# arangesh/TrackMPNN

Hardware: AMD Instinct MI355X
Metric: graph_edges_per_sec_fwd_bwd (higher is better)
Workload: dtype f32; 1 GPU; C2 KITTI Car/RRC-shaped rolling windows: 7 frames, D_t~clip(Poisson(6),1,20), F=8 (2d), H=64, K=0, diff; 1 fwd per frame + 1 bwd per window; 16384 windows/GPU batched block-diagonally (64 distinct seeds tiled); windows_per_gpu=16384, rows_final=6762496, parallelism=sequence-dp1

## Files before the change

### trackmpnn_amd/csrc/intf.hip

```cpp
#include "common.h"
#include <stdlib.h>

namespace tmpnn {

static constexpr float IT_EPS = 1e-5f;
static constexpr int IT_CH = 128;
static constexpr int IT_SPB = 32;
static constexpr int IT_FMAX = 128;
static constexpr int IT_NT = 1024;

struct ItFwdArgs {
    const float* x; const int64_t* x_rows; int ld_x; int F; int nd;
    const int32_t* seg_ptr; const int32_t* seg_cnt; const int32_t* seg_of_det; int S; int training;
    const float* w1; const float* b1; const float* gamma; const float* beta;
    const float* run_mean; const float* run_var; const float* w2; const float* b2;
    float* y_save; float* mean; float* rstd; const int32_t* out_row; float* h_new; int ld_h;
};

__device__ __forceinline__ int it_chunk_end(const int* s_sp, int s0, int sa, int s1) {
    const int base = s_sp[sa - s0];
    int sb = sa + 1;
    while (sb < s1 && s_sp[sb + 1 - s0] - base <= IT_CH) ++sb;
    return sb;
}

template <int H>
__global__ __launch_bounds__(IT_NT) void k_it_fwd(ItFwdArgs a) {
    constexpr int NSUB = IT_NT / H, LD = H + 4;
    extern __shared__ __attribute__((aligned(16))) float it_lds[];
    float* s_w2 = it_lds;
    float* s_y = s_w2 + H * LD;
    float* s_a = s_y + IT_CH * LD;
    float* s_mean = s_a + IT_CH * LD;
    float* s_rstd = s_mean + IT_SPB * H;
    float* s_w1 = s_rstd + IT_SPB * H;
    float* s_x = s_w1;
    const int tid = threadIdx.x, c = tid % H, sub = tid / H;
    const int F = a.F;
    for (int i = tid; i < H * H; i += IT_NT) s_w2[(i / H) * LD + (i % H)] = a.w2[i];
    float w1r[16];
    if (F <= 16) {
#pragma unroll
        for (int f = 0; f < 16; ++f) w1r[f] = f < F ? a.w1[c * F + f] : 0.f;
    } else {
        for (int i = tid; i < H * F; i += IT_NT) s_w1[(i / F) * (F + 1) + (i % F)] = a.w1[i];
    }
    const float b1 = a.b1[c], gam = a.gamma[c], bet = a.beta[c], b2 = a.b2[c];
    __shared__ int s_sp[IT_SPB + 1];
    if (!a.training) {
        if (sub == 0) {
            const float m = a.run_mean[c], r = rsqrtf(a.run_var[c] + IT_EPS);
            s_mean[c] = m; s_rstd[c] = r;
            if (blockIdx.x == 0) { a.mean[c] = m; a.rstd[c] = r; }
        }
    }
    const int ngroups = a.training ? (a.S + IT_SPB - 1) / IT_SPB : (a.nd + IT_CH - 1) / IT_CH;
    for (int grp = blockIdx.x; grp < ngroups; grp += gridDim.x) {
    int s0, s1;
    if (a.training) { s0 = grp * IT_SPB; s1 = min(a.S, s0 + IT_SPB); }
    else { s0 = grp; s1 = s0 + 1; }
    __syncthreads();
    if (a.training && tid <= s1 - s0) s_sp[tid] = a.seg_ptr[s0 + tid];
    __syncthreads();
    for (int sa = s0; sa < s1;) {
        int sb, ra, rb;
        if (a.training) { sb = it_chunk_end(s_sp, s0, sa, s1); ra = s_sp[sa - s0]; rb = s_sp[sb - s0]; }
        else { sb = s1; ra = sa * IT_CH; rb = min(a.nd, ra + IT_CH); }
        const int nr = rb - ra;
        if (F <= 16) {
            for (int t = tid; t < nr * 16; t += IT_NT) {
                const int i = t >> 4, f = t & 15;
                const size_t xrow = a.x_rows ? (size_t)a.x_rows[ra + i] : (size_t)(ra + i);
                s_x[t] = f < F ? a.x[xrow * a.ld_x + f] : 0.f;
            }
            __syncthreads();
        }
        for (int i = sub; i < nr; i += NSUB) {
            const float* xr = a.x + ((F > 16 && a.x_rows) ? (size_t)a.x_rows[ra + i] : (size_t)(ra + i)) * a.ld_x;
            float acc = b1;
            if (F <= 16) {
#pragma unroll
                for (int f4 = 0; f4 < 4; ++f4) {
                    const float4 xv = *reinterpret_cast<const float4*>(s_x + i * 16 + 4 * f4);
                    acc = fmaf(xv.x, w1r[4 * f4], acc); acc = fmaf(xv.y, w1r[4 * f4 + 1], acc);
                    acc = fmaf(xv.z, w1r[4 * f4 + 2], acc); acc = fmaf(xv.w, w1r[4 * f4 + 3], acc);
                }
            } else {
                for (int f = 0; f < F; ++f) acc = fmaf(xr[f], s_w1[c * (F + 1) + f], acc);
            }
            s_y[i * LD + c] = acc;
            a.y_save[(size_t)(ra + i) * H + c] = acc;
        }
        __syncthreads();
        if (a.training) {
            for (int s = sa + sub; s < sb; s += NSUB) {
                const int p0 = s_sp[s - s0] - ra, p1 = s_sp[s + 1 - s0] - ra;
                const float cnt = (float)a.seg_cnt[s], nz = cnt - (float)(p1 - p0);
                float sum = nz * b1;
                for (int i = p0; i < p1; ++i) sum += s_y[i * LD + c];
                const float m = sum / cnt;
                float sq = nz * (b1 - m) * (b1 - m);
                for (int i = p0; i < p1; ++i) { const float d = s_y[i * LD + c] - m; sq += d * d; }
                const float r = rsqrtf(sq / cnt + IT_EPS);
                s_mean[(s - sa) * H + c] = m; s_rstd[(s - sa) * H + c] = r;
                a.mean[(size_t)s * H + c] = m; a.rstd[(size_t)s * H + c] = r;
            }
            __syncthreads();
        }
        for (int i = sub; i < nr; i += NSUB) {
            int sl = 0;
            if (a.training) { while (s_sp[sa - s0 + sl + 1] - ra <= i) ++sl; }
            const float yh = (s_y[i * LD + c] - s_mean[sl * H + c]) * s_rstd[sl * H + c];
            s_a[i * LD + c] = fmaxf(yh * gam + bet, 0.f);
        }
        __syncthreads();
        for (int i0 = sub; i0 < nr; i0 += 4 * NSUB) {
            float acc[4] = {b2, b2, b2, b2};
            int rr[4], orow[4];
#pragma unroll
            for (int t = 0; t < 4; ++t) rr[t] = min(i0 + t * NSUB, nr - 1);
#pragma unroll
            for (int t = 0; t < 4; ++t) orow[t] = a.out_row[ra + rr[t]];
#pragma unroll 4
            for (int k4 = 0; k4 < H / 4; ++k4) {
                const float4 w = *reinterpret_cast<const float4*>(s_w2 + c * LD + 4 * k4);
#pragma unroll
                for (int t = 0; t < 4; ++t) {
                    const float4 av = *reinterpret_cast<const float4*>(s_a + rr[t] * LD + 4 * k4);
                    acc[t] = fmaf(av.x, w.x, acc[t]); acc[t] = fmaf(av.y, w.y, acc[t]);
                    acc[t] = fmaf(av.z, w.z, acc[t]); acc[t] = fmaf(av.w, w.w, acc[t]);
                }
            }
#pragma unroll
            for (int t = 0; t < 4; ++t) {
                const int i = i0 + t * NSUB;
                if (i < nr) a.h_new[(size_t)orow[t] * a.ld_h + c] = acc[t];
            }
        }
        __syncthreads();
        sa = sb;
    }
    }
}

struct ItBwdArgs {
    const float* x; const int64_t* x_rows; int ld_x; int F; int nd;
    const int32_t* seg_ptr; const int32_t* seg_cnt; const int32_t* seg_of_det; int S; int training;
    const float* w1; const float* b1; const float* gamma; const float* beta; const float* w2;
    const float* y_save; const float* mean; const float* rstd; const int32_t* out_row;
    const float* d_h; int ld_dh; float* d_xdet; int ld_dx; float* d_xzero;
    float* slabs; int slab_floats;
};

template <int H, int FPT>
__global__ __launch_bounds__(IT_NT) void k_it_bwd(ItBwdArgs a) {
    constexpr int NSUB = IT_NT / H, LD = H + 4, KPT = H / NSUB;
    extern __shared__ __attribute__((aligned(16))) float it_lds[];
    float* s_w2 = it_lds;
    float* s_d = s_w2 + H * LD;
    float* s_a = s_d + IT_CH * LD;
    float* s_yh = s_a + IT_CH * LD;
    float* s_dy0 = s_yh + IT_CH * LD;
    float* s_red = s_dy0 + IT_SPB * H;
    float* s_x = s_red + 4 * IT_NT;
    float* s_w1 = s_x + IT_CH * 16;
    const int tid = threadIdx.x, c = tid % H, sub = tid / H;
    const int F = a.F;
    for (int i = tid; i < H * H; i += IT_NT) s_w2[(i % H) * LD + (i / H)] = a.w2[i];
    if (F <= 16)
        for (int i = tid; i < H * 16; i += IT_NT) s_w1[(i >> 4) * 17 + (i & 15)] = (i & 15) < F ? a.w1[(i >> 4) * F + (i & 15)] : 0.f;
    const float b1 = a.b1[c], gam = a.gamma[c], bet = a.beta[c];
    float acc_w2[KPT];
#pragma unroll
    for (int j = 0; j < KPT; ++j) acc_w2[j] = 0.f;
    float acc_w1[FPT];
#pragma unroll
    for (int j = 0; j < FPT; ++j) acc_w1[j] = 0.f;
    float v_db2 = 0.f, v_dg = 0.f, v_dbt = 0.f, v_db1 = 0.f;
    __shared__ int s_sp[IT_SPB + 1];
    const int ngroups = a.training ? (a.S + IT_SPB - 1) / IT_SPB : (a.nd + IT_CH - 1) / IT_CH;
    for (int grp = blockIdx.x; grp < ngroups; grp += gridDim.x) {
    int s0, s1;
    if (a.training) { s0 = grp * IT_SPB; s1 = min(a.S, s0 + IT_SPB); }
    else { s0 = grp; s1 = s0 + 1; }
    __syncthreads();
    if (a.training && tid <= s1 - s0) s_sp[tid] = a.seg_ptr[s0 + tid];
    __syncthreads();
    for (int sa = s0; sa < s1;) {
        int sb, ra, rb;
        if (a.training) { sb = it_chunk_end(s_sp, s0, sa, s1); ra = s_sp[sa - s0]; rb = s_sp[sb - s0]; }
        else { sb = s1; ra = sa * IT_CH; rb = min(a.nd, ra + IT_CH); }
        const int nr = rb - ra;
        {
            constexpr int RPT = IT_CH / NSUB;
            int orow[RPT], sg[RPT];
#pragma unroll
            for (int j = 0; j < RPT; ++j) {
                const int i = min(sub + j * NSUB, nr - 1);
                orow[j] = a.out_row[ra + i];
                int sl = 0;
                if (a.training) { while (s_sp[sa - s0 + sl + 1] - ra <= i) ++sl; }
                sg[j] = a.training ? sa + sl : 0;
            }
            float dv[RPT], yv[RPT], mv[RPT], rv[RPT];
#pragma unroll
            for (int j = 0; j < RPT; ++j) {
                const int i = min(sub + j * NSUB, nr - 1);
                dv[j] = a.d_h[(size_t)orow[j] * a.ld_dh + c];
                yv[j] = a.y_save[(size_t)(ra + i) * H + c];
                mv[j] = a.mean[(size_t)sg[j] * H + c];
                rv[j] = a.rstd[(size_t)sg[j] * H + c];
            }
#pragma unroll
            for (int j = 0; j < RPT; ++j) {
                const int i = sub + j * NSUB;
                if (i < nr) {
                    const float yh = (yv[j] - mv[j]) * rv[j];
                    s_yh[i * LD + c] = yh;
                    s_a[i * LD + c] = fmaxf(yh * gam + bet, 0.f);
                    s_d[i * LD + c] = dv[j];
                }
            }
        }
        if (F <= 16) {
            for (int t = tid; t < nr * 16; t += IT_NT) {
                const int i = t >> 4, f = t & 15;
                const size_t xrow = a.x_rows ? (size_t)a.x_rows[ra + i] : (size_t)(ra + i);
                s_x[t] = f < F ? a.x[xrow * a.ld_x + f] : 0.f;
            }
        }
        __syncthreads();
#pragma unroll 8
        for (int i = 0; i < nr; ++i) {
            const float d = s_d[i * LD + c];
            if (sub == 0) v_db2 += d;
            if constexpr (KPT % 4 == 0) {
#pragma unroll
                for (int j4 = 0; j4 < KPT / 4; ++j4) {
                    const float4 av = *reinterpret_cast<const float4*>(s_a + i * LD + KPT * sub + 4 * j4);
                    acc_w2[4 * j4 + 0] = fmaf(d, av.x, acc_w2[4 * j4 + 0]); acc_w2[4 * j4 + 1] = fmaf(d, av.y, acc_w2[4 * j4 + 1]);
                    acc_w2[4 * j4 + 2] = fmaf(d, av.z, acc_w2[4 * j4 + 2]); acc_w2[4 * j4 + 3] = fmaf(d, av.w, acc_w2[4 * j4 + 3]);
                }
            } else {
#pragma unroll
                for (int j = 0; j < KPT; ++j) acc_w2[j] = fmaf(d, s_a[i * LD + KPT * sub + j], acc_w2[j]);
            }
        }
        __syncthreads();
        for (int i0 = sub; i0 < nr; i0 += 4 * NSUB) {
            float da[4] = {0.f, 0.f, 0.f, 0.f};
            int rr[4];
#pragma unroll
            for (int t = 0; t < 4; ++t) rr[t] = min(i0 + t * NSUB, nr - 1);
#pragma unroll 4
            for (int c4 = 0; c4 < H / 4; ++c4) {
                const float4 w = *reinterpret_cast<const float4*>(s_w2 + c * LD + 4 * c4);
#pragma unroll
                for (int t = 0; t < 4; ++t) {
                    const float4 dv = *reinterpret_cast<const float4*>(s_d + rr[t] * LD + 4 * c4);
                    da[t] = fmaf(dv.x, w.x, da[t]); da[t] = fmaf(dv.y, w.y, da[t]);
                    da[t] = fmaf(dv.z, w.z, da[t]); da[t] = fmaf(dv.w, w.w, da[t]);
                }
            }
            float dyh[4];
#pragma unroll
            for (int t = 0; t < 4; ++t) {
                const int i = i0 + t * NSUB;
                dyh[t] = 0.f;
                if (i < nr) {
                    const float dz = s_a[i * LD + c] > 0.f ? da[t] : 0.f;
                    v_dg = fmaf(dz, s_yh[i * LD + c], v_dg);
                    v_dbt += dz;
                    dyh[t] = dz * gam;
                }
            }
#pragma unroll
            for (int t = 0; t < 4; ++t) {
                const int i = i0 + t * NSUB;
                if (i < nr) s_a[i * LD + c] = dyh[t];
            }
        }
        __syncthreads();
        if (a.training) {
            for (int s = sa + sub; s < sb; s += NSUB) {
                const int p0 = s_sp[s - s0] - ra, p1 = s_sp[s + 1 - s0] - ra;
                const float cnt = (float)a.seg_cnt[s], nz = cnt - (float)(p1 - p0);
                const float m = a.mean[(size_t)s * H + c], r = a.rstd[(size_t)s * H + c];
                float q1 = 0.f, q2 = 0.f;
                for (int i = p0; i < p1; ++i) { const float g = s_a[i * LD + c]; q1 += g; q2 = fmaf(g, s_yh[i * LD + c], q2); }
                const float inv = 1.0f / cnt;
                for (int i = p0; i < p1; ++i) {
                    const float dy = r * (s_a[i * LD + c] - q1 * inv - s_yh[i * LD + c] * q2 * inv);
                    s_a[i * LD + c] = dy;
                    v_db1 += dy;
                }
                const float yh0 = (b1 - m) * r;
                const float dy0 = r * (-q1 * inv - yh0 * q2 * inv);
                v_db1 = fmaf(nz, dy0, v_db1);
                s_dy0[(s - sa) * H + c] = dy0;
            }
        } else {
            const float r = a.rstd[c];
            for (int i = sub; i < nr; i += NSUB) { const float dy = r * s_a[i * LD + c]; s_a[i * LD + c] = dy; v_db1 += dy; }
        }
        __syncthreads();
        if (F <= 16) {
#pragma unroll 4
            for (int i = 0; i < nr; ++i) {
                const float dy = s_a[i * LD + c];
#pragma unroll
                for (int j = 0; j < (FPT < 4 ? FPT : 4); ++j) {
                    const int f = sub + j * NSUB;
                    if (f < 16) acc_w1[j] = fmaf(dy, s_x[i * 16 + f], acc_w1[j]);
                }
            }
        } else {
            for (int i = 0; i < nr; ++i) {
                const float dy = s_a[i * LD + c];
                const float* xr = a.x + (a.x_rows ? (size_t)a.x_rows[ra + i] : (size_t)(ra + i)) * a.ld_x;
#pragma unroll
                for (int j = 0; j < FPT; ++j) {
                    const int f = sub + j * NSUB;
                    if (f < F) acc_w1[j] = fmaf(dy, xr[f], acc_w1[j]);
                }
            }
        }
        if (a.d_xdet) {
            for (int t = tid; t < nr * F; t += IT_NT) {
                const int i = t / F, f = t - i * F;
                float acc = 0.f;
                if (F <= 16) {
#pragma unroll 8
                    for (int k = 0; k < H; ++k) acc = fmaf(s_a[i * LD + k], s_w1[k * 17 + f], acc);
                } else {
                    for (int k = 0; k < H; ++k) acc = fmaf(s_a[i * LD + k], a.w1[k * F + f], acc);
                }
                a.d_xdet[(size_t)(ra + i) * a.ld_dx + f] = acc;
            }
        }
        if (a.d_xzero && a.training) {
            const int ns = sb - sa;
            for (int t = tid; t < ns * F; t += IT_NT) {
                const int s = t / F, f = t - s * F;
                float acc = 0.f;
                if (F <= 16) {
#pragma unroll 8
                    for (int k = 0; k < H; ++k) acc = fmaf(s_dy0[s * H + k], s_w1[k * 17 + f], acc);
                } else {
                    for (int k = 0; k < H; ++k) acc = fmaf(s_dy0[s * H + k], a.w1[k * F + f], acc);
                }
                a.d_xzero[(size_t)(sa + s) * F + f] = acc;
            }
        }
        __syncthreads();
        sa = sb;
    }
    }
    float* slab = a.slabs + (size_t)blockIdx.x * a.slab_floats;
#pragma unroll
    for (int j = 0; j < KPT; ++j) slab[c * H + KPT * sub + j] = acc_w2[j];
    float* sl_w1 = slab + H * H;
#pragma unroll
    for (int j = 0; j < FPT; ++j) {
        const int f = sub + j * NSUB;
        if (f < F) sl_w1[c * F + f] = acc_w1[j];
    }
    s_red[0 * IT_NT + tid] = v_db2; s_red[1 * IT_NT + tid] = v_dg; s_red[2 * IT_NT + tid] = v_dbt; s_red[3 * IT_NT + tid] = v_db1;
    __syncthreads();
    if (sub == 0) {
        float* sl_v = sl_w1 + H * F;
#pragma unroll
        for (int q = 0; q < 4; ++q) {
            float v = 0.f;
            for (int t = 0; t < NSUB; ++t) v += s_red[q * IT_NT + t * H + c];
            sl_v[q * H + c] = v;
        }
    }
}

static constexpr int ITW_R = 32;
static constexpr int ITW_MS = 8;
static constexpr int ITW_NW = 8;
static constexpr int ITW_SPB = 64;
static constexpr int ITW_FWD_WAVE_FLOATS = ITW_R * 64 + ITW_R * 16;
static constexpr int ITW_BWD_WAVE_FLOATS = 2 * ITW_R * 64 + ITW_R * 16;

#define ITW_LDS_SYNC() asm volatile("s_waitcnt lgkmcnt(0)" ::: "memory")
__device__ __forceinline__ int itw_chunk_end(const int* s_sp, int s0, int sa, int s1) {
    const int base = s_sp[sa - s0];
    int sb = sa + 1;
    while (sb < s1 && sb - sa < ITW_MS && s_sp[sb + 1 - s0] - base <= ITW_R) ++sb;
    return sb;
}

__device__ __forceinline__ void itw_stage_x(const float* __restrict__ x, const int64_t* __restrict__ x_rows, int ld_x, int F,
                                            int ra, int nr, int lane, float* s_x) {
    size_t xrow[8];
#pragma unroll
    for (int q = 0; q < 8; ++q) {
        const int t = lane + 64 * q, i = min(t >> 4, nr - 1);
        xrow[q] = x_rows ? (size_t)x_rows[ra + i] : (size_t)(ra + i);
    }
    float v[8];
#pragma unroll
    for (int q = 0; q < 8; ++q) {
        const int f = lane & 15;
        v[q] = x[xrow[q] * ld_x + min(f, F - 1)];
    }
#pragma unroll
    for (int q = 0; q < 8; ++q) {
        const int t = lane + 64 * q;
        if (t < nr * 16) s_x[t] = (lane & 15) < F ? v[q] : 0.f;
    }
}

__device__ __forceinline__ float itw_col_sum(const float* col, int p0, int p1) {
    float sum = 0.f;
    for (int b = p0; b < p1; b += 8) {
        float v[8];
#pragma unroll
        for (int t = 0; t < 8; ++t) v[t] = col[min(b + t, p1 - 1) * 64];
#pragma unroll
        for (int t = 0; t < 8; ++t) sum += (b + t < p1) ? v[t] : 0.f;
    }
    return sum;
}

__global__ __launch_bounds__(ITW_NW * 64) void k_itw_fwd(ItFwdArgs a) {
    constexpr int H = 64;
    extern __shared__ __attribute__((aligned(16))) float it_lds[];
    __shared__ int s_sp[ITW_SPB + 1];
    const int tid = threadIdx.x, c = tid & 63, wave = tid >> 6;
    float* s_a = it_lds + wave * ITW_FWD_WAVE_FLOATS;
    float* s_x = s_a + ITW_R * 64;
    float* col = s_a + c;
    const int F = a.F;
    float w1r[16], w2r[64];
#pragma unroll
    for (int f = 0; f < 16; ++f) w1r[f] = f < F ? a.w1[c * F + f] : 0.f;
#pragma unroll
    for (int k4 = 0; k4 < 16; ++k4) {
        const float4 w = *reinterpret_cast<const float4*>(a.w2 + c * H + 4 * k4);
        w2r[4 * k4] = w.x; w2r[4 * k4 + 1] = w.y; w2r[4 * k4 + 2] = w.z; w2r[4 * k4 + 3] = w.w;
    }
    const float b1 = a.b1[c], gam = a.gamma[c], bet = a.beta[c], b2 = a.b2[c];
    const int ngroups = (a.S + ITW_SPB - 1) / ITW_SPB;
    for (int grp = blockIdx.x; grp < ngroups; grp += gridDim.x) {
        const int s0 = grp * ITW_SPB, s1 = min(a.S, s0 + ITW_SPB);
        __syncthreads();
        if (tid <= s1 - s0) s_sp[tid] = a.seg_ptr[s0 + tid];
        __syncthreads();
        const int nxt_l = (s0 + c < s1) ? itw_chunk_end(s_sp, s0, s0 + c, s1) : s1;
        int j = 0;
        for (int sa = s0; sa < s1; ++j) {
            const int sb = __shfl(nxt_l, sa - s0, 64);
            if ((j & (ITW_NW - 1)) == wave) {
                const int ra = s_sp[sa - s0], nr = s_sp[sb - s0] - ra;
                int orow_l = 0, cnt_l = 1;
                if (c < nr) orow_l = a.out_row[ra + c];
                if (sa + c < sb) cnt_l = a.seg_cnt[sa + c];
                if (nr > 0) {
                    itw_stage_x(a.x, a.x_rows, a.ld_x, F, ra, nr, c, s_x);
                    ITW_LDS_SYNC();
                    for (int i = 0; i < nr; i += 2) {
                        const int i1 = min(i + 1, nr - 1);
                        float acc0 = b1, acc1 = b1;
#pragma unroll
                        for (int f4 = 0; f4 < 4; ++f4) {
                            const float4 x0 = *reinterpret_cast<const float4*>(s_x + i * 16 + 4 * f4);
                            const float4 x1 = *reinterpret_cast<const float4*>(s_x + i1 * 16 + 4 * f4);
                            acc0 = fmaf(x0.x, w1r[4 * f4], acc0); acc0 = fmaf(x0.y, w1r[4 * f4 + 1], acc0);
                            acc0 = fmaf(x0.z, w1r[4 * f4 + 2], acc0); acc0 = fmaf(x0.w, w1r[4 * f4 + 3], acc0);
                            acc1 = fmaf(x1.x, w1r[4 * f4], acc1); acc1 = fmaf(x1.y, w1r[4 * f4 + 1], acc1);
                            acc1 = fmaf(x1.z, w1r[4 * f4 + 2], acc1); acc1 = fmaf(x1.w, w1r[4 * f4 + 3], acc1);
                        }
                        col[i * 64] = acc0;
                        a.y_save[(size_t)(ra + i) * H + c] = acc0;
                        if (i + 1 < nr) { col[i1 * 64] = acc1; a.y_save[(size_t)(ra + i1) * H + c] = acc1; }
                    }
                }
                for (int s = sa; s < sb; ++s) {
                    const int p0 = s_sp[s - s0] - ra, p1 = s_sp[s + 1 - s0] - ra;
                    const float cnt = (float)__shfl(cnt_l, s - sa, 64), nz = cnt - (float)(p1 - p0);
                    const float m = (nz * b1 + itw_col_sum(col, p0, p1)) / cnt;
                    float sq = nz * (b1 - m) * (b1 - m);
                    for (int b = p0; b < p1; b += 8) {
                        float v[8];
#pragma unroll
                        for (int t = 0; t < 8; ++t) v[t] = col[min(b + t, p1 - 1) * 64];
#pragma unroll
                        for (int t = 0; t < 8; ++t) { const float d = v[t] - m; sq += (b + t < p1) ? d * d : 0.f; }
                    }
                    const float r = rsqrtf(sq / cnt + IT_EPS);
                    a.mean[(size_t)s * H + c] = m; a.rstd[(size_t)s * H + c] = r;
                    for (int b = p0; b < p1; b += 8) {
                        float v[8];
#pragma unroll
                        for (int t = 0; t < 8; ++t) v[t] = col[min(b + t, p1 - 1) * 64];
#pragma unroll
                        for (int t = 0; t < 8; ++t)
                            if (b + t < p1) col[(b + t) * 64] = fmaxf((v[t] - m) * r * gam + bet, 0.f);
                    }
                }
                ITW_LDS_SYNC();
                for (int i = 0; i < nr; i += 2) {
                    const int i1 = min(i + 1, nr - 1);
                    float acc0 = b2, acc1 = b2;
#pragma unroll
                    for (int k4 = 0; k4 < 16; ++k4) {
                        const float4 a0 = *reinterpret_cast<const float4*>(s_a + i * 64 + 4 * k4);
                        const float4 a1 = *reinterpret_cast<const float4*>(s_a + i1 * 64 + 4 * k4);
                        acc0 = fmaf(a0.x, w2r[4 * k4], acc0); acc0 = fmaf(a0.y, w2r[4 * k4 + 1], acc0);
                        acc0 = fmaf(a0.z, w2r[4 * k4 + 2], acc0); acc0 = fmaf(a0.w, w2r[4 * k4 + 3], acc0);
                        acc1 = fmaf(a1.x, w2r[4 * k4], acc1); acc1 = fmaf(a1.y, w2r[4 * k4 + 1], acc1);
                        acc1 = fmaf(a1.z, w2r[4 * k4 + 2], acc1); acc1 = fmaf(a1.w, w2r[4 * k4 + 3], acc1);
                    }
                    const int o0 = __shfl(orow_l, i, 64), o1 = __shfl(orow_l, i1, 64);
                    a.h_new[(size_t)o0 * a.ld_h + c] = acc0;
                    if (i + 1 < nr) a.h_new[(size_t)o1 * a.ld_h + c] = acc1;
                }
                ITW_LDS_SYNC();
            }
            sa = sb;
        }
    }
}

__global__ __launch_bounds__(ITW_NW * 64) void k_itw_bwd(ItBwdArgs a) {
    constexpr int H = 64;
    extern __shared__ __attribute__((aligned(16))) float it_lds[];
    __shared__ int s_sp[ITW_SPB + 1];
    const int tid = threadIdx.x, c = tid & 63, wave = tid >> 6;
    float* s_yh = it_lds + wave * ITW_BWD_WAVE_FLOATS;
    float* s_d = s_yh + ITW_R * 64;
    float* s_x = s_d + ITW_R * 64;
    float* cyh = s_yh + c;
    float* cd = s_d + c;
    const int F = a.F;
    float w2c[64];
#pragma unroll
    for (int j = 0; j < 64; ++j) w2c[j] = a.w2[j * H + c];
    const float b1 = a.b1[c], gam = a.gamma[c], bet = a.beta[c];
    float acc_w2t[64];
#pragma unroll
    for (int j = 0; j < 64; ++j) acc_w2t[j] = 0.f;
    float acc_w1[16];
#pragma unroll
    for (int f = 0; f < 16; ++f) acc_w1[f] = 0.f;
    float v_dg = 0.f, v_dbt = 0.f, v_db1 = 0.f;
    float v_db2 = 0.f;
    const int ngroups = (a.S + ITW_SPB - 1) / ITW_SPB;
    for (int grp = blockIdx.x; grp < ngroups; grp += gridDim.x) {
        const int s0 = grp * ITW_SPB, s1 = min(a.S, s0 + ITW_SPB);
        __syncthreads();
        if (tid <= s1 - s0) s_sp[tid] = a.seg_ptr[s0 + tid];
        __syncthreads();
        const int nxt_l = (s0 + c < s1) ? itw_chunk_end(s_sp, s0, s0 + c, s1) : s1;
        int j = 0;
        for (int sa = s0; sa < s1; ++j) {
            const int sb = __shfl(nxt_l, sa - s0, 64);
            if ((j & (ITW_NW - 1)) == wave) {
                const int ra = s_sp[sa - s0], nr = s_sp[sb - s0] - ra;
                int orow_l = 0, cnt_l = 1;
                if (c < nr) orow_l = a.out_row[ra + c];
                if (sa + c < sb) cnt_l = a.seg_cnt[sa + c];
                float mseg[ITW_MS], rseg[ITW_MS];
#pragma unroll
                for (int t = 0; t < ITW_MS; ++t) {
                    const int s = min(sa + t, sb - 1);
                    mseg[t] = a.mean[(size_t)s * H + c];
                    rseg[t] = a.rstd[(size_t)s * H + c];
                }
                if (nr > 0) itw_stage_x(a.x, a.x_rows, a.ld_x, F, ra, nr, c, s_x);
                for (int b = 0; b < nr; b += 8) {
                    float dv[8], yv[8];
#pragma unroll
                    for (int t = 0; t < 8; ++t) {
                        const int i = min(b + t, nr - 1);
                        const int orow = __shfl(orow_l, i, 64);
                        dv[t] = a.d_h[(size_t)orow * a.ld_dh + c];
                        yv[t] = a.y_save[(size_t)(ra + i) * H + c];
                    }
#pragma unroll
                    for (int t = 0; t < 8; ++t) {
                        if (b + t < nr) { cd[(b + t) * 64] = dv[t]; cyh[(b + t) * 64] = yv[t]; v_db2 += dv[t]; }
                    }
                }
#pragma unroll
                for (int t = 0; t < ITW_MS; ++t) {
                    if (sa + t < sb) {
                        const int p0 = s_sp[sa + t - s0] - ra, p1 = s_sp[sa + t + 1 - s0] - ra;
                        for (int b = p0; b < p1; b += 8) {
                            float v[8];
#pragma unroll
                            for (int u = 0; u < 8; ++u) v[u] = cyh[min(b + u, p1 - 1) * 64];
#pragma unroll
                            for (int u = 0; u < 8; ++u)
                                if (b + u < p1) cyh[(b + u) * 64] = (v[u] - mseg[t]) * rseg[t];
                        }
                    }
                }
                ITW_LDS_SYNC();
                for (int i = 0; i < nr; ++i) {
                    const float yh = cyh[i * 64];
                    const float av = fmaxf(yh * gam + bet, 0.f);
                    float da0 = 0.f, da1 = 0.f;
#pragma unroll
                    for (int j4 = 0; j4 < 16; ++j4) {
                        const float4 dv = *reinterpret_cast<const float4*>(s_d + i * 64 + 4 * j4);
                        acc_w2t[4 * j4] = fmaf(dv.x, av, acc_w2t[4 * j4]); acc_w2t[4 * j4 + 1] = fmaf(dv.y, av, acc_w2t[4 * j4 + 1]);
                        acc_w2t[4 * j4 + 2] = fmaf(dv.z, av, acc_w2t[4 * j4 + 2]); acc_w2t[4 * j4 + 3] = fmaf(dv.w, av, acc_w2t[4 * j4 + 3]);
                        da0 = fmaf(dv.x, w2c[4 * j4], da0); da1 = fmaf(dv.y, w2c[4 * j4 + 1], da1);
                        da0 = fmaf(dv.z, w2c[4 * j4 + 2], da0); da1 = fmaf(dv.w, w2c[4 * j4 + 3], da1);
                    }
                    const float dz = av > 0.f ? da0 + da1 : 0.f;
                    v_dg = fmaf(dz, yh, v_dg);
                    v_dbt += dz;
                    ITW_LDS_SYNC();
                    cd[i * 64] = dz * gam;
                }
#pragma unroll
                for (int t = 0; t < ITW_MS; ++t) {
                    if (sa + t < sb) {
                        const int p0 = s_sp[sa + t - s0] - ra, p1 = s_sp[sa + t + 1 - s0] - ra;
                        const float cnt = (float)__shfl(cnt_l, t, 64), nz = cnt - (float)(p1 - p0);
                        const float m = mseg[t], r = rseg[t];
                        float q1 = 0.f, q2 = 0.f;
                        for (int b = p0; b < p1; b += 8) {
                            float g[8], y[8];
#pragma unroll
                            for (int u = 0; u < 8; ++u) { const int i = min(b + u, p1 - 1); g[u] = cd[i * 64]; y[u] = cyh[i * 64]; }
#pragma unroll
                            for (int u = 0; u < 8; ++u)
                                if (b + u < p1) { q1 += g[u]; q2 = fmaf(g[u], y[u], q2); }
                        }
                        const float inv = 1.0f / cnt;
                        for (int b = p0; b < p1; b += 8) {
                            float g[8], y[8];
#pragma unroll
                            for (int u = 0; u < 8; ++u) { const int i = min(b + u, p1 - 1); g[u] = cd[i * 64]; y[u] = cyh[i * 64]; }
#pragma unroll
                            for (int u = 0; u < 8; ++u) {
                                if (b + u < p1) {
                                    const float dy = r * (g[u] - q1 * inv - y[u] * q2 * inv);
                                    cd[(b + u) * 64] = dy;
                                    v_db1 += dy;
                                }
                            }
                        }
                        const float yh0 = (b1 - m) * r;
                        const float dy0 = r * (-q1 * inv - yh0 * q2 * inv);
                        v_db1 = fmaf(nz, dy0, v_db1);
                    }
                }
                for (int i = 0; i < nr; i += 2) {
                    const int i1 = min(i + 1, nr - 1);
                    const float dy0 = cd[i * 64], dy1 = (i + 1 < nr) ? cd[i1 * 64] : 0.f;
#pragma unroll
                    for (int f4 = 0; f4 < 4; ++f4) {
                        const float4 x0 = *reinterpret_cast<const float4*>(s_x + i * 16 + 4 * f4);
                        const float4 x1 = *reinterpret_cast<const float4*>(s_x + i1 * 16 + 4 * f4);
                        acc_w1[4 * f4] = fmaf(dy0, x0.x, acc_w1[4 * f4]); acc_w1[4 * f4 + 1] = fmaf(dy0, x0.y, acc_w1[4 * f4 + 1]);
                        acc_w1[4 * f4 + 2] = fmaf(dy0, x0.z, acc_w1[4 * f4 + 2]); acc_w1[4 * f4 + 3] = fmaf(dy0, x0.w, acc_w1[4 * f4 + 3]);
                        acc_w1[4 * f4] = fmaf(dy1, x1.x, acc_w1[4 * f4]); acc_w1[4 * f4 + 1] = fmaf(dy1, x1.y, acc_w1[4 * f4 + 1]);
                        acc_w1[4 * f4 + 2] = fmaf(dy1, x1.z, acc_w1[4 * f4 + 2]); acc_w1[4 * f4 + 3] = fmaf(dy1, x1.w, acc_w1[4 * f4 + 3]);
                    }
                }
                ITW_LDS_SYNC();
            }
            sa = sb;
        }
    }
    __syncthreads();
    float* s_all = it_lds;
    float* mine = s_all + wave * ITW_BWD_WAVE_FLOATS;
#pragma unroll
    for (int j = 0; j < 64; ++j) mine[j * 64 + c] = acc_w2t[j];
    __syncthreads();
    float* slab = a.slabs + (size_t)blockIdx.x * a.slab_floats;
    for (int e = tid; e < H * H; e += ITW_NW * 64) {
        float v = 0.f;
#pragma unroll
        for (int w = 0; w < ITW_NW; ++w) v += s_all[w * ITW_BWD_WAVE_FLOATS + e];
        slab[e] = v;
    }
    __syncthreads();
#pragma unroll
    for (int f = 0; f < 16; ++f) mine[c * 16 + f] = acc_w1[f];
    mine[1024 + c] = v_db2; mine[1088 + c] = v_dg; mine[1152 + c] = v_dbt; mine[1216 + c] = v_db1;
    __syncthreads();
    float* sl_w1 = slab + H * H;
    for (int e = tid; e < H * F; e += ITW_NW * 64) {
        const int k = e / F, f = e - k * F;
        float v = 0.f;
#pragma unroll
        for (int w = 0; w < ITW_NW; ++w) v += s_all[w * ITW_BWD_WAVE_FLOATS + k * 16 + f];
        sl_w1[e] = v;
    }
    float* sl_v = sl_w1 + H * F;
    for (int e = tid; e < 4 * H; e += ITW_NW * 64) {
        float v = 0.f;
#pragma unroll
        for (int w = 0; w < ITW_NW; ++w) v += s_all[w * ITW_BWD_WAVE_FLOATS + 1024 + e];
        sl_v[e] = v;
    }
}

static bool itw_serves(int H, int F, int max_seg_rows, int training) {
    static const int off = [] { const char* e = getenv("TMPNN_IT_WAVE"); return (e && e[0] == '0') ? 1 : 0; }();
    return !off && training && H == 64 && F <= 16 && max_seg_rows <= ITW_R;
}
static int itw_blocks(int S) {
    const int groups = ceil_div(S, ITW_SPB);
    int dev = 0, cus = 256;
    if (hipGetDevice(&dev) == hipSuccess) (void)hipDeviceGetAttribute(&cus, hipDeviceAttributeMultiprocessorCount, dev);
    return groups < cus ? groups : cus;
}

__global__ __launch_bounds__(256) void k_it_reduce(const float* __restrict__ slabs, int nslab, int slab_floats, int H, int F,
                                                   float* dw2, float* dw1, float* db2, float* dgamma, float* dbeta, float* db1) {
    __shared__ float s_part[8][32];
    const int el = threadIdx.x & 31, slice = threadIdx.x >> 5;
    const int e = blockIdx.x * 32 + el;
    const int n_w2 = H * H, n_w1 = H * F, total = n_w2 + n_w1 + 4 * H;
    const int per = (nslab + 7) / 8;
    const int sl0 = slice * per, sl1 = min(nslab, sl0 + per);
    float v = 0.f;
    if (e < total)
        for (int s = sl0; s < sl1; ++s) v += slabs[(size_t)s * slab_floats + e];
    s_part[slice][el] = v;
    __syncthreads();
    if (slice != 0 || e >= total) return;
    float sum = 0.f;
#pragma unroll
    for (int q = 0; q < 8; ++q) sum += s_part[q][el];
    if (e < n_w2) dw2[e] += sum;
    else if (e < n_w2 + n_w1) dw1[e - n_w2] += sum;
    else {
        const int q = (e - n_w2 - n_w1) / H, j = (e - n_w2 - n_w1) % H;
        (q == 0 ? db2 : q == 1 ? dgamma : q == 2 ? dbeta : db1)[j] += sum;
    }
}

__global__ __launch_bounds__(64) void k_it_running(const float* __restrict__ mean, const float* __restrict__ rstd,
                                                   const int32_t* __restrict__ seg_cnt, int S, int H,
                                                   float* __restrict__ rm, float* __restrict__ rv) {
    const int j = blockIdx.x, lane = threadIdx.x;
    const int s0 = S > 320 ? S - 320 : 0;
    float m = 0.f, v = 0.f;
    for (int s = s0 + lane; s < S; s += 64) {
        const float w = 0.1f * powf(0.9f, (float)(S - 1 - s));
        const float cnt = (float)seg_cnt[s];
        const float r = rstd[(size_t)s * H + j];
        const float var = 1.0f / (r * r) - IT_EPS;
        m += w * mean[(size_t)s * H + j];
        v += w * var * (cnt / (cnt - 1.0f));
    }
    for (int off = 32; off >= 1; off >>= 1) { m += __shfl_xor(m, off); v += __shfl_xor(v, off); }
    if (lane == 0) {
        const float keep = s0 > 0 ? 0.f : powf(0.9f, (float)S);
        rm[j] = keep * rm[j] + m;
        rv[j] = keep * rv[j] + v;
    }
}

static size_t it_fwd_shm(int H, int F) {
    return sizeof(float) * ((size_t)H * (H + 4) + 2 * (size_t)IT_CH * (H + 4) + 2 * (size_t)IT_SPB * H +
                            (F > 16 ? (size_t)H * (F + 1) : (size_t)IT_CH * 16));
}
static size_t it_bwd_shm(int H) {
    return sizeof(float) * ((size_t)H * (H + 4) + 3 * (size_t)IT_CH * (H + 4) + (size_t)IT_SPB * H + 4 * IT_NT + (size_t)IT_CH * 16 +
                            (size_t)H * 17);
}
static int it_blocks(int nd, int S, int training) {
    const int groups = training ? ceil_div(S, IT_SPB) : ceil_div(nd, IT_CH);
    int dev = 0, cus = 256;
    if (hipGetDevice(&dev) == hipSuccess) (void)hipDeviceGetAttribute(&cus, hipDeviceAttributeMultiprocessorCount, dev);
    return groups < cus ? groups : cus;
}

}

using namespace tmpnn;

extern "C" {

int tmpnn_input_tf_supported(int H, int F, int max_seg_rows) {
    return ((H == 32 || H == 64) && F > 0 && F <= IT_FMAX && max_seg_rows >= 0 && max_seg_rows <= IT_CH) ? 1 : 0;
}

int tmpnn_input_tf_fwd(const float* xdet, const int64_t* x_rows, int ld_x, int F, int nd, const int32_t* seg_ptr, const int32_t* seg_cnt,
                       const int32_t* seg_of_det, int S, int max_seg_rows, int H, int training, const float* w1, const float* b1,
                       const float* gamma, const float* beta, float* running_mean, float* running_var, const float* w2,
                       const float* b2, float* y_save, float* mean, float* rstd, const int32_t* out_row, float* h_new,
                       int ld_h, tmpnn_stream stream) {
    TM_REQUIRE(tmpnn_input_tf_supported(H, F, max_seg_rows), "input_tf_fwd: H=%d F=%d max_seg_rows=%d (H in {32, 64}, F <= %d, "
               "segments of at most %d det rows; use tmpnn_input_bn_fwd otherwise)", H, F, max_seg_rows, IT_FMAX, IT_CH);
    TM_REQUIRE(nd >= 0 && S >= 0, "input_tf_fwd: nd=%d S=%d", nd, S);
    TM_REQUIRE(w1 && b1 && gamma && beta && running_mean && running_var && w2 && b2 && mean && rstd, "input_tf_fwd: null parameter pointer");
    TM_REQUIRE(!training || (seg_ptr && seg_cnt && seg_of_det && S > 0), "input_tf_fwd: training needs segments");
    hipStream_t st = as_stream(stream);
    if (nd == 0 && !training) return TMPNN_OK;
    TM_REQUIRE(nd == 0 || (xdet && y_save && out_row && h_new && ld_x >= F && ld_h >= H), "input_tf_fwd: null/short buffers");
    ItFwdArgs a{xdet, x_rows, ld_x, F, nd, seg_ptr, seg_cnt, seg_of_det, S, training, w1, b1, gamma, beta, running_mean, running_var,
                w2, b2, y_save, mean, rstd, out_row, h_new, ld_h};
    if (nd > 0 && itw_serves(H, F, max_seg_rows, training)) {
        const size_t shmw = sizeof(float) * (size_t)ITW_NW * ITW_FWD_WAVE_FLOATS;
        TM_SHM_ONCE(k_itw_fwd, shmw);
        hipLaunchKernelGGL(k_itw_fwd, dim3(itw_blocks(S)), dim3(ITW_NW * 64), shmw, st, a);
        int rc = check_launch("itw_fwd");
        if (rc) return rc;
        hipLaunchKernelGGL(k_it_running, dim3(H), dim3(64), 0, st, mean, rstd, seg_cnt, S, H, running_mean, running_var);
        return check_launch("it_running");
    }
    const int nb = it_blocks(nd, S, training);
    const size_t shm = it_fwd_shm(H, F);
    if (nb > 0) {
        if (H == 64) { TM_SHM_ONCE(k_it_fwd<64>, it_fwd_shm(64, IT_FMAX)); hipLaunchKernelGGL(k_it_fwd<64>, dim3(nb), dim3(IT_NT), shm, st, a); }
        else { TM_SHM_ONCE(k_it_fwd<32>, it_fwd_shm(32, IT_FMAX)); hipLaunchKernelGGL(k_it_fwd<32>, dim3(nb), dim3(IT_NT), shm, st, a); }
        int rc = check_launch("it_fwd");
        if (rc) return rc;
    }
    if (training) {
        hipLaunchKernelGGL(k_it_running, dim3(H), dim3(64), 0, st, mean, rstd, seg_cnt, S, H, running_mean, running_var);
        return check_launch("it_running");
    }
    return TMPNN_OK;
}

size_t tmpnn_input_tf_bwd_ws(int nd, int S, int H, int F, int training) {
    int nb = it_blocks(nd, S, training);
    if (training && itw_blocks(S) > nb) nb = itw_blocks(S);
    return sizeof(float) * (size_t)(nb > 0 ? nb : 1) * ((size_t)H * H + (size_t)H * F + 4 * H);
}

int tmpnn_input_tf_bwd(const float* xdet, const int64_t* x_rows, int ld_x, int F, int nd, const int32_t* seg_ptr, const int32_t* seg_cnt,
                       const int32_t* seg_of_det, int S, int max_seg_rows, int H, int training, const float* w1, const float* b1,
                       const float* gamma, const float* beta, const float* w2, const float* y_save, const float* mean,
                       const float* rstd, const int32_t* out_row, const float* d_h, int ld_dh, float* d_xdet, int ld_dx,
                       float* d_xzero, float* dw1, float* db1, float* dgamma, float* dbeta, float* dw2, float* db2, void* ws,
                       size_t ws_bytes, tmpnn_stream stream) {
    TM_REQUIRE(tmpnn_input_tf_supported(H, F, max_seg_rows), "input_tf_bwd: H=%d F=%d max_seg_rows=%d", H, F, max_seg_rows);
    TM_REQUIRE(nd >= 0 && S >= 0, "input_tf_bwd: nd=%d S=%d", nd, S);
    TM_REQUIRE(w1 && b1 && gamma && beta && w2 && mean && rstd && dw1 && db1 && dgamma && dbeta && dw2 && db2, "input_tf_bwd: null parameter pointer");
    hipStream_t st = as_stream(stream);
    if (nd == 0) {
        if (d_xzero && S > 0) (void)hipMemsetAsync(d_xzero, 0, sizeof(float) * (size_t)S * F, st);
        return TMPNN_OK;
    }
    TM_REQUIRE(xdet && y_save && out_row && d_h && ws, "input_tf_bwd: null buffers");
    TM_REQUIRE(!training || (seg_ptr && seg_cnt && seg_of_det && S > 0), "input_tf_bwd: training needs segments");
    const size_t need = tmpnn_input_tf_bwd_ws(nd, S, H, F, training);
    if (ws_bytes < need) return set_error(TMPNN_EWORKSPACE, "input_tf_bwd: workspace %zu < %zu bytes", ws_bytes, need);
    if (!training && d_xzero && S > 0) (void)hipMemsetAsync(d_xzero, 0, sizeof(float) * (size_t)S * F, st);
    const bool wave_form = itw_serves(H, F, max_seg_rows, training) && d_xdet == nullptr && d_xzero == nullptr;
    const int nb = wave_form ? itw_blocks(S) : it_blocks(nd, S, training);
    const int slab_floats = H * H + H * F + 4 * H;
    ItBwdArgs a{xdet, x_rows, ld_x, F, nd, seg_ptr, seg_cnt, seg_of_det, S, training, w1, b1, gamma, beta, w2, y_save, mean, rstd, out_row,
                d_h, ld_dh, d_xdet, ld_dx, d_xzero, reinterpret_cast<float*>(ws), slab_floats};
    if (wave_form) {
        const size_t shmw = sizeof(float) * (size_t)ITW_NW * ITW_BWD_WAVE_FLOATS;
        TM_SHM_ONCE(k_itw_bwd, shmw);
        hipLaunchKernelGGL(k_itw_bwd, dim3(nb), dim3(ITW_NW * 64), shmw, st, a);
        int rc = check_launch("itw_bwd");
        if (rc) return rc;
        hipLaunchKernelGGL(k_it_reduce, dim3(ceil_div(slab_floats, 32)), dim3(256), 0, st, reinterpret_cast<const float*>(ws), nb,
                           slab_floats, H, F, dw2, dw1, db2, dgamma, dbeta, db1);
        return check_launch("it_reduce");
    }
#define IT_BWD(HH, FF)                                                                                   \
    do {                                                                                                 \
        TM_SHM_ONCE((k_it_bwd<HH, FF>), it_bwd_shm(HH));                                                 \
        hipLaunchKernelGGL((k_it_bwd<HH, FF>), dim3(nb), dim3(IT_NT), it_bwd_shm(HH), st, a);              \
    } while (0)
    if (H == 64) { if (F <= 16) IT_BWD(64, 1); else IT_BWD(64, IT_FMAX / 16); }
    else { if (F <= 16) IT_BWD(32, 1); else IT_BWD(32, IT_FMAX / 32); }
#undef IT_BWD
    int rc = check_launch("it_bwd");
    if (rc) return rc;
    hipLaunchKernelGGL(k_it_reduce, dim3(ceil_div(slab_floats, 32)), dim3(256), 0, st, reinterpret_cast<const float*>(ws), nb,
                       slab_floats, H, F, dw2, dw1, db2, dgamma, dbeta, db1);
    return check_launch("it_reduce");
}

}
```

Before: 731.1 million graph-edges/s.

## Use MFMA 32x32x2 f32 for second linear layer forward and backward in windowed kernels

Replaces the per-lane scalar FMA loops for the 64x64 second linear layer with MFMA f32 32x32x2 instructions. This covers the forward output, the backward input gradient and the weight-gradient accumulation. LDS activation rows are padded to a stride of 68 to avoid bank conflicts on the row-major reads the MFMA operands need. The backward pass is split into an MFMA gradient phase followed by a separate ReLU/BN-gradient pass, and the weight registers shrink from 64 per lane to a 2x32 tile. This adds more LDS traffic for scattering the MFMA results and raises the per-wave LDS footprint.

```diff
diff --git a/trackmpnn_amd/csrc/intf.hip b/trackmpnn_amd/csrc/intf.hip
--- a/trackmpnn_amd/csrc/intf.hip
+++ b/trackmpnn_amd/csrc/intf.hip
@@ -382,10 +382,14 @@
 static constexpr int ITW_MS = 8;
 static constexpr int ITW_NW = 8;
 static constexpr int ITW_SPB = 64;
-static constexpr int ITW_FWD_WAVE_FLOATS = ITW_R * 64 + ITW_R * 16;
-static constexpr int ITW_BWD_WAVE_FLOATS = 2 * ITW_R * 64 + ITW_R * 16;
+static constexpr int ITW_LD = 68;
+static constexpr int ITW_FWD_WAVE_FLOATS = ITW_R * ITW_LD + ITW_R * 16;
+static constexpr int ITW_BWD_WAVE_FLOATS = ITW_R * 64 + ITW_R * ITW_LD + ITW_R * 16;
+static_assert(ITW_BWD_WAVE_FLOATS >= 64 * 64, "the slab combine stages a wave's 64 x 64 accumulators in its own area");
 
 #define ITW_LDS_SYNC() asm volatile("s_waitcnt lgkmcnt(0)" ::: "memory")
+__device__ __forceinline__ f32x16 itw_mfma(float a, float b, f32x16 c) { return __builtin_amdgcn_mfma_f32_32x32x2f32(a, b, c, 0, 0, 0); }
+__device__ __forceinline__ int itw_drow(int r, int lane) { return 8 * (r >> 2) + 4 * (lane >> 5) + (r & 3); }
 __device__ __forceinline__ int itw_chunk_end(const int* s_sp, int s0, int sa, int s1) {
     const int base = s_sp[sa - s0];
     int sb = sa + 1;
@@ -419,7 +423,7 @@
     for (int b = p0; b < p1; b += 8) {
         float v[8];
 #pragma unroll
-        for (int t = 0; t < 8; ++t) v[t] = col[min(b + t, p1 - 1) * 64];
+        for (int t = 0; t < 8; ++t) v[t] = col[min(b + t, p1 - 1) * ITW_LD];
 #pragma unroll
         for (int t = 0; t < 8; ++t) sum += (b + t < p1) ? v[t] : 0.f;
     }
@@ -432,18 +436,23 @@
     __shared__ int s_sp[ITW_SPB + 1];
     const int tid = threadIdx.x, c = tid & 63, wave = tid >> 6;
     float* s_a = it_lds + wave * ITW_FWD_WAVE_FLOATS;
-    float* s_x = s_a + ITW_R * 64;
+    float* s_x = s_a + ITW_R * ITW_LD;
     float* col = s_a + c;
     const int F = a.F;
-    float w1r[16], w2r[64];
+    const int cl = c & 31, cg = c >> 5;
+    float w1r[16];
 #pragma unroll
     for (int f = 0; f < 16; ++f) w1r[f] = f < F ? a.w1[c * F + f] : 0.f;
-#pragma unroll
-    for (int k4 = 0; k4 < 16; ++k4) {
-        const float4 w = *reinterpret_cast<const float4*>(a.w2 + c * H + 4 * k4);
-        w2r[4 * k4] = w.x; w2r[4 * k4 + 1] = w.y; w2r[4 * k4 + 2] = w.z; w2r[4 * k4 + 3] = w.w;
-    }
-    const float b1 = a.b1[c], gam = a.gamma[c], bet = a.beta[c], b2 = a.b2[c];
+    float w2r[2][32];
+#pragma unroll
+    for (int nb = 0; nb < 2; ++nb)
+#pragma unroll
+        for (int k4 = 0; k4 < 8; ++k4) {
+            const float4 w = *reinterpret_cast<const float4*>(a.w2 + (cl + 32 * nb) * H + 32 * cg + 4 * k4);
+            w2r[nb][4 * k4] = w.x; w2r[nb][4 * k4 + 1] = w.y; w2r[nb][4 * k4 + 2] = w.z; w2r[nb][4 * k4 + 3] = w.w;
+        }
+    const float b1 = a.b1[c], gam = a.gamma[c], bet = a.beta[c];
+    const float b2lo = a.b2[cl], b2hi = a.b2[cl + 32];
     const int ngroups = (a.S + ITW_SPB - 1) / ITW_SPB;
     for (int grp = blockIdx.x; grp < ngroups; grp += gridDim.x) {
         const int s0 = grp * ITW_SPB, s1 = min(a.S, s0 + ITW_SPB);
@@ -474,9 +483,9 @@
                             acc1 = fmaf(x1.x, w1r[4 * f4], acc1); acc1 = fmaf(x1.y, w1r[4 * f4 + 1], acc1);
                             acc1 = fmaf(x1.z, w1r[4 * f4 + 2], acc1); acc1 = fmaf(x1.w, w1r[4 * f4 + 3], acc1);
                         }
-                        col[i * 64] = acc0;
+                        col[i * ITW_LD] = acc0;
                         a.y_save[(size_t)(ra + i) * H + c] = acc0;
-                        if (i + 1 < nr) { col[i1 * 64] = acc1; a.y_save[(size_t)(ra + i1) * H + c] = acc1; }
+                        if (i + 1 < nr) { col[i1 * ITW_LD] = acc1; a.y_save[(size_t)(ra + i1) * H + c] = acc1; }
                     }
                 }
                 for (int s = sa; s < sb; ++s) {
@@ -487,7 +496,7 @@
                     for (int b = p0; b < p1; b += 8) {
                         float v[8];
 #pragma unroll
-                        for (int t = 0; t < 8; ++t) v[t] = col[min(b + t, p1 - 1) * 64];
+                        for (int t = 0; t < 8; ++t) v[t] = col[min(b + t, p1 - 1) * ITW_LD];
 #pragma unroll
                         for (int t = 0; t < 8; ++t) { const float d = v[t] - m; sq += (b + t < p1) ? d * d : 0.f; }
                     }
@@ -496,28 +505,35 @@
                     for (int b = p0; b < p1; b += 8) {
                         float v[8];
 #pragma unroll
-                        for (int t = 0; t < 8; ++t) v[t] = col[min(b + t, p1 - 1) * 64];
+                        for (int t = 0; t < 8; ++t) v[t] = col[min(b + t, p1 - 1) * ITW_LD];
 #pragma unroll
                         for (int t = 0; t < 8; ++t)
-                            if (b + t < p1) col[(b + t) * 64] = fmaxf((v[t] - m) * r * gam + bet, 0.f);
+                            if (b + t < p1) col[(b + t) * ITW_LD] = fmaxf((v[t] - m) * r * gam + bet, 0.f);
                     }
                 }
                 ITW_LDS_SYNC();
-                for (int i = 0; i < nr; i += 2) {
-                    const int i1 = min(i + 1, nr - 1);
-                    float acc0 = b2, acc1 = b2;
-#pragma unroll
-                    for (int k4 = 0; k4 < 16; ++k4) {
-                        const float4 a0 = *reinterpret_cast<const float4*>(s_a + i * 64 + 4 * k4);
-                        const float4 a1 = *reinterpret_cast<const float4*>(s_a + i1 * 64 + 4 * k4);
-                        acc0 = fmaf(a0.x, w2r[4 * k4], acc0); acc0 = fmaf(a0.y, w2r[4 * k4 + 1], acc0);
-                        acc0 = fmaf(a0.z, w2r[4 * k4 + 2], acc0); acc0 = fmaf(a0.w, w2r[4 * k4 + 3], acc0);
-                        acc1 = fmaf(a1.x, w2r[4 * k4], acc1); acc1 = fmaf(a1.y, w2r[4 * k4 + 1], acc1);
-                        acc1 = fmaf(a1.z, w2r[4 * k4 + 2], acc1); acc1 = fmaf(a1.w, w2r[4 * k4 + 3], acc1);
-                    }
-                    const int o0 = __shfl(orow_l, i, 64), o1 = __shfl(orow_l, i1, 64);
-                    a.h_new[(size_t)o0 * a.ld_h + c] = acc0;
-                    if (i + 1 < nr) a.h_new[(size_t)o1 * a.ld_h + c] = acc1;
+                if (nr > 0) {
+                    f32x16 o0, o1;
+#pragma unroll
+                    for (int r = 0; r < 16; ++r) { o0[r] = b2lo; o1[r] = b2hi; }
+                    const float* arow = s_a + cl * ITW_LD + 32 * cg;
+#pragma unroll
+                    for (int q = 0; q < 8; ++q) {
+                        const float4 av = *reinterpret_cast<const float4*>(arow + 4 * q);
+                        o0 = itw_mfma(av.x, w2r[0][4 * q], o0); o1 = itw_mfma(av.x, w2r[1][4 * q], o1);
+                        o0 = itw_mfma(av.y, w2r[0][4 * q + 1], o0); o1 = itw_mfma(av.y, w2r[1][4 * q + 1], o1);
+                        o0 = itw_mfma(av.z, w2r[0][4 * q + 2], o0); o1 = itw_mfma(av.z, w2r[1][4 * q + 2], o1);
+                        o0 = itw_mfma(av.w, w2r[0][4 * q + 3], o0); o1 = itw_mfma(av.w, w2r[1][4 * q + 3], o1);
+                    }
+#pragma unroll
+                    for (int r = 0; r < 16; ++r) {
+                        const int i = itw_drow(r, c);
+                        const int o = __shfl(orow_l, i, 64);
+                        if (i < nr) {
+                            float* dst = a.h_new + (size_t)o * a.ld_h + cl;
+                            dst[0] = o0[r]; dst[32] = o1[r];
+                        }
+                    }
                 }
                 ITW_LDS_SYNC();
             }
@@ -533,17 +549,21 @@
     const int tid = threadIdx.x, c = tid & 63, wave = tid >> 6;
     float* s_yh = it_lds + wave * ITW_BWD_WAVE_FLOATS;
     float* s_d = s_yh + ITW_R * 64;
-    float* s_x = s_d + ITW_R * 64;
+    float* s_x = s_d + ITW_R * ITW_LD;
     float* cyh = s_yh + c;
     float* cd = s_d + c;
     const int F = a.F;
-    float w2c[64];
-#pragma unroll
-    for (int j = 0; j < 64; ++j) w2c[j] = a.w2[j * H + c];
+    const int cl = c & 31, cg = c >> 5;
+    float w2b[2][32];
+#pragma unroll
+    for (int nb = 0; nb < 2; ++nb)
+#pragma unroll
+        for (int t = 0; t < 32; ++t) w2b[nb][t] = a.w2[(32 * cg + t) * H + cl + 32 * nb];
     const float b1 = a.b1[c], gam = a.gamma[c], bet = a.beta[c];
-    float acc_w2t[64];
-#pragma unroll
-    for (int j = 0; j < 64; ++j) acc_w2t[j] = 0.f;
+    const float gam_lo = a.gamma[cl], gam_hi = a.gamma[cl + 32], bet_lo = a.beta[cl], bet_hi = a.beta[cl + 32];
+    f32x16 acc_w2[2][2];
+#pragma unroll
+    for (int r = 0; r < 16; ++r) { acc_w2[0][0][r] = 0.f; acc_w2[0][1][r] = 0.f; acc_w2[1][0][r] = 0.f; acc_w2[1][1][r] = 0.f; }
     float acc_w1[16];
 #pragma unroll
     for (int f = 0; f < 16; ++f) acc_w1[f] = 0.f;
@@ -583,7 +603,7 @@
                     }
 #pragma unroll
                     for (int t = 0; t < 8; ++t) {
-                        if (b + t < nr) { cd[(b + t) * 64] = dv[t]; cyh[(b + t) * 64] = yv[t]; v_db2 += dv[t]; }
+                        if (b + t < nr) { cd[(b + t) * ITW_LD] = dv[t]; cyh[(b + t) * 64] = yv[t]; v_db2 += dv[t]; }
                     }
                 }
 #pragma unroll
@@ -601,23 +621,52 @@
                     }
                 }
                 ITW_LDS_SYNC();
-                for (int i = 0; i < nr; ++i) {
-                    const float yh = cyh[i * 64];
-                    const float av = fmaxf(yh * gam + bet, 0.f);
-                    float da0 = 0.f, da1 = 0.f;
-#pragma unroll
-                    for (int j4 = 0; j4 < 16; ++j4) {
-                        const float4 dv = *reinterpret_cast<const float4*>(s_d + i * 64 + 4 * j4);
-                        acc_w2t[4 * j4] = fmaf(dv.x, av, acc_w2t[4 * j4]); acc_w2t[4 * j4 + 1] = fmaf(dv.y, av, acc_w2t[4 * j4 + 1]);
-                        acc_w2t[4 * j4 + 2] = fmaf(dv.z, av, acc_w2t[4 * j4 + 2]); acc_w2t[4 * j4 + 3] = fmaf(dv.w, av, acc_w2t[4 * j4 + 3]);
-                        da0 = fmaf(dv.x, w2c[4 * j4], da0); da1 = fmaf(dv.y, w2c[4 * j4 + 1], da1);
-                        da0 = fmaf(dv.z, w2c[4 * j4 + 2], da0); da1 = fmaf(dv.w, w2c[4 * j4 + 3], da1);
-                    }
-                    const float dz = av > 0.f ? da0 + da1 : 0.f;
-                    v_dg = fmaf(dz, yh, v_dg);
-                    v_dbt += dz;
+                if (nr > 0) {
+                    const int nt = (nr + 1) >> 1;
+                    const float* dcol = s_d + cg * ITW_LD + cl;
+                    const float* ycol = s_yh + cg * 64 + cl;
+                    for (int t = 0; t < nt; ++t) {
+                        const bool live = 2 * t + cg < nr;
+                        const float d0 = dcol[2 * t * ITW_LD], d1 = dcol[2 * t * ITW_LD + 32];
+                        const float y0 = ycol[2 * t * 64], y1 = ycol[2 * t * 64 + 32];
+                        const float a0 = live ? fmaxf(y0 * gam_lo + bet_lo, 0.f) : 0.f, a1 = live ? fmaxf(y1 * gam_hi + bet_hi, 0.f) : 0.f;
+                        const float e0 = live ? d0 : 0.f, e1 = live ? d1 : 0.f;
+                        acc_w2[0][0] = itw_mfma(e0, a0, acc_w2[0][0]); acc_w2[0][1] = itw_mfma(e0, a1, acc_w2[0][1]);
+                        acc_w2[1][0] = itw_mfma(e1, a0, acc_w2[1][0]); acc_w2[1][1] = itw_mfma(e1, a1, acc_w2[1][1]);
+                    }
+                    f32x16 da0, da1;
+#pragma unroll
+                    for (int r = 0; r < 16; ++r) { da0[r] = 0.f; da1[r] = 0.f; }
+                    const float* drow = s_d + cl * ITW_LD + 32 * cg;
+#pragma unroll
+                    for (int q = 0; q < 8; ++q) {
+                        const float4 dv = *reinterpret_cast<const float4*>(drow + 4 * q);
+                        da0 = itw_mfma(dv.x, w2b[0][4 * q], da0); da1 = itw_mfma(dv.x, w2b[1][4 * q], da1);
+                        da0 = itw_mfma(dv.y, w2b[0][4 * q + 1], da0); da1 = itw_mfma(dv.y, w2b[1][4 * q + 1], da1);
+                        da0 = itw_mfma(dv.z, w2b[0][4 * q + 2], da0); da1 = itw_mfma(dv.z, w2b[1][4 * q + 2], da1);
+                        da0 = itw_mfma(dv.w, w2b[0][4 * q + 3], da0); da1 = itw_mfma(dv.w, w2b[1][4 * q + 3], da1);
+                    }
+#pragma unroll
+                    for (int r = 0; r < 16; ++r) {
+                        float* dst = s_d + itw_drow(r, c) * ITW_LD + cl;
+                        dst[0] = da0[r]; dst[32] = da1[r];
+                    }
                     ITW_LDS_SYNC();
-                    cd[i * 64] = dz * gam;
+                }
+                for (int b = 0; b < nr; b += 8) {
+                    float g[8], y[8];
+#pragma unroll
+                    for (int u = 0; u < 8; ++u) { const int i = min(b + u, nr - 1); g[u] = cd[i * ITW_LD]; y[u] = cyh[i * 64]; }
+#pragma unroll
+                    for (int u = 0; u < 8; ++u) {
+                        if (b + u < nr) {
+                            const float av = fmaxf(y[u] * gam + bet, 0.f);
+                            const float dz = av > 0.f ? g[u] : 0.f;
+                            v_dg = fmaf(dz, y[u], v_dg);
+                            v_dbt += dz;
+                            cd[(b + u) * ITW_LD] = dz * gam;
+                        }
+                    }
                 }
 #pragma unroll
                 for (int t = 0; t < ITW_MS; ++t) {
@@ -629,7 +678,7 @@
                         for (int b = p0; b < p1; b += 8) {
                             float g[8], y[8];
 #pragma unroll
-                            for (int u = 0; u < 8; ++u) { const int i = min(b + u, p1 - 1); g[u] = cd[i * 64]; y[u] = cyh[i * 64]; }
+                            for (int u = 0; u < 8; ++u) { const int i = min(b + u, p1 - 1); g[u] = cd[i * ITW_LD]; y[u] = cyh[i * 64]; }
 #pragma unroll
                             for (int u = 0; u < 8; ++u)
                                 if (b + u < p1) { q1 += g[u]; q2 = fmaf(g[u], y[u], q2); }
@@ -638,12 +687,12 @@
                         for (int b = p0; b < p1; b += 8) {
                             float g[8], y[8];
 #pragma unroll
-                            for (int u = 0; u < 8; ++u) { const int i = min(b + u, p1 - 1); g[u] = cd[i * 64]; y[u] = cyh[i * 64]; }
+                            for (int u = 0; u < 8; ++u) { const int i = min(b + u, p1 - 1); g[u] = cd[i * ITW_LD]; y[u] = cyh[i * 64]; }
 #pragma unroll
                             for (int u = 0; u < 8; ++u) {
                                 if (b + u < p1) {
                                     const float dy = r * (g[u] - q1 * inv - y[u] * q2 * inv);
-                                    cd[(b + u) * 64] = dy;
+                                    cd[(b + u) * ITW_LD] = dy;
                                     v_db1 += dy;
                                 }
                             }
@@ -655,7 +704,7 @@
                 }
                 for (int i = 0; i < nr; i += 2) {
                     const int i1 = min(i + 1, nr - 1);
-                    const float dy0 = cd[i * 64], dy1 = (i + 1 < nr) ? cd[i1 * 64] : 0.f;
+                    const float dy0 = cd[i * ITW_LD], dy1 = (i + 1 < nr) ? cd[i1 * ITW_LD] : 0.f;
 #pragma unroll
                     for (int f4 = 0; f4 < 4; ++f4) {
                         const float4 x0 = *reinterpret_cast<const float4*>(s_x + i * 16 + 4 * f4);
@@ -675,7 +724,11 @@
     float* s_all = it_lds;
     float* mine = s_all + wave * ITW_BWD_WAVE_FLOATS;
 #pragma unroll
-    for (int j = 0; j < 64; ++j) mine[j * 64 + c] = acc_w2t[j];
+    for (int r = 0; r < 16; ++r) {
+        float* dst = mine + itw_drow(r, c) * 64 + cl;
+        dst[0] = acc_w2[0][0][r]; dst[32] = acc_w2[0][1][r];
+        dst[32 * 64] = acc_w2[1][0][r]; dst[32 * 64 + 32] = acc_w2[1][1][r];
+    }
     __syncthreads();
     float* slab = a.slabs + (size_t)blockIdx.x * a.slab_floats;
     for (int e = tid; e < H * H; e += ITW_NW * 64) {
```

Result: no change. 731.1 million graph-edges/s (median of 3 runs) (-0.0%).
